# joshspeagle/brutus

Measured on AMD Instinct MI355X. Metric: stars/sec at 750k-model x 12-band grid; achieved HBM GB/s vs peak, higher is better.
Workload: dtype f64; 1 GPU; configs[1]: 750k-model x 12-band grid, Av-only solve (rvlim=(3.32,3.32)), no parallax; grid = synth.make_mist_like_grid (lattice-ordered like the MIST grid files); grid_generator=mist_like, nmodel=750000, nfilt=12, sub_batch=128, selected_models_last_sub_batch=44670752, streams_per_gpu=3, parallelism=stars sharded, 1 rank(s), no data-path collective

## Files before the change

brutus_amd/csrc/fit2_kernels.hpp:

```cpp
#pragma once

#include "fit_kernels.hpp"
#include "pre32_types.hpp"

namespace {

static_assert(PS_TILE == TILE && PS_NBMAX == NBMAX, "pre32_types.hpp and common.hpp disagree");

struct CallInit {
    int32_t *ids_all, *kfix, *k2, *counters;
    int ncounters;
};
__global__ void __launch_bounds__(64)
k_prep32(int nstar, const StarPrep *__restrict__ stars, float eps_scale, int dim_prior,
         Star32 *__restrict__ out, CallInit init) {
    static_assert(NBMAX <= 64, "one lane per band");
    __shared__ double s_a[NBMAX], s_b[NBMAX], s_c[NBMAX];
    __shared__ double s_gbar, s_D;
    __shared__ int s_bad;
    const int s = blockIdx.x, j = threadIdx.x;
    if (s >= nstar) return;
    if (init.ids_all && j == 0) {
        init.ids_all[s] = s;
        init.kfix[s] = 2;
// ... 316 lines not shown
            const float x = fmaxf(fmaxf(slot[0][threadIdx.x], slot[1][threadIdx.x]),
                                  fmaxf(slot[2][threadIdx.x], slot[3][threadIdx.x]));
            part[((int64_t)bx * nstar + s) * NV32 + v] = x;
        }
    }
}

__global__ void k_pre_decide(int nblkx, int nstar, const int32_t *__restrict__ star_ids,
                             const float *__restrict__ part, const Star32 *__restrict__ stars,
                             float ln_init, int rvf, int32_t *kfix,
                             int accept, float *__restrict__ st32, int32_t *__restrict__ k1,
                             int32_t *__restrict__ status, double *__restrict__ nomA,
                             int32_t *ctr, int32_t *__restrict__ probe_ids,
                             int32_t *__restrict__ redo_ids, const int32_t *nrun_dev) {
    __shared__ float sm[NV32][4];
    if (nrun_dev && (int)blockIdx.x >= *nrun_dev) return;
    const int s = star_ids[blockIdx.x];
    float v[NV32];
    for (int q = 0; q < NV32; ++q) v[q] = -INFINITY;
    for (int b = threadIdx.x; b < nblkx; b += blockDim.x) {
        const float *pp = part + ((int64_t)b * nstar + s) * NV32;
        for (int q = 0; q < NV32; ++q) v[q] = fmaxf(v[q], pp[q]);
    }
    for (int q = 0; q < NV32; ++q) {
        float x = v[q];
        for (int off = 32; off > 0; off >>= 1) x = fmaxf(x, __shfl_xor(x, off, 64));
        if ((threadIdx.x & 63) == 0) sm[q][threadIdx.x >> 6] = x;
    }
    __syncthreads();
    if (threadIdx.x != 0) return;
    for (int q = 0; q < NV32; ++q)
        v[q] = fmaxf(fmaxf(sm[q][0], sm[q][1]), fmaxf(sm[q][2], sm[q][3]));
    for (int q = 0; q < NV32; ++q) st32[(int64_t)s * NV32 + q] = v[q];
    const Star32 &sp = stars[s];
    const float ew = 2.f * sp.epsw;
    int st = 2, K1 = 0;
    const int K = kfix[s];
    if (sp.ok && !(v[8] > 0.f) && v[0] > -INFINITY) {
        const bool cont1 = v[1] > v[0] + ln_init + ew;
        const bool may1 = v[2] > v[0] + ln_init - ew;
        if (!may1) {
            K1 = 1;
            st = (rvf || K == 1) ? 0 : 1;
        } else if (cont1) {
            if (rvf) {
                K1 = 2;
                st = 0;
            } else if (K >= 2) {
                const bool cont2 = v[4] > v[3] + ln_init + ew;
                const bool may2 = v[5] > v[3] + ln_init - ew;
                if (!may2) {
                    K1 = 2;
                    st = (K == 2) ? 0 : 2;
                } else if (cont2) {
                    st = 2;
                }
            }
        }
    }
    if (!accept) {
        k1[s] = K1;
        status[s] = st;
        if (ctr) {
            if (st == 1) {
                kfix[s] = K1;
                redo_ids[atomicAdd(ctr + 1, 1)] = s;
            } else if (st == 2) {
                probe_ids[atomicAdd(ctr + 0, 1)] = s;
            }
        }
    }
    nomA[s] = (double)v[6] - 2. * (double)sp.eps;
}

template <int NB, bool RVF>
struct Tile64 {
    Coef<NB> c;
    double F0[NB];
    double R[RVF ? NB : 1];
};

template <int NB, bool RVF>
__device__ __forceinline__ void tile_load(const float *__restrict__ grid, int64_t nmodel_pad,
                                          int64_t i, double rv_mean, Tile64<NB, RVF> &t) {
    load_coef<NB>(grid, nmodel_pad, i, t.c);
    load_F0<NB>(grid, nmodel_pad, i, t.F0);
    if constexpr (RVF) coef_R<NB>(t.c, rv_mean, t.R);
}

template <int NB, bool RVF>
__device__ __forceinline__ void mag_phase(const Tile64<NB, RVF> &t, const StarPrep &sp,
                                          const DevParams &p, int K, double &av, double &rv) {
    av = p.av_mean;
    rv = p.rv_mean;
    if constexpr (RVF) {
        GramR Gm;
        gram_init_rf<NB>(t.c, t.R, sp, Gm);
        double a_, c_;
        if (K > 0) gram_sweep_rf(Gm, sp.S, p, av, a_, c_);
    } else {
        Gram Gm;
        gram_init<NB>(t.c, sp, Gm);
        for (int k = 0; k < K; ++k) {
            double a_, b_, c_;
            gram_sweep(Gm, sp.S, p, av, rv, a_, b_, c_);
        }
    }
}

template <int NB, bool RVF, bool FULL>
__device__ __forceinline__ void mle_at(const Tile64<NB, RVF> &t, const StarPrep &sp,
                                       const DevParams &p, double av, double rv,
                                       const double *__restrict__ tbl, Mle &m) {
    if constexpr (RVF) mle_fast_rf<NB, true, FULL ? 2 : 0>(t.c, t.R, t.F0, sp, p, av, tbl, m);
    else mle_fast<NB, true, FULL ? 2 : 0>(t.c, t.F0, sp, p, av, rv, tbl, m);
}

__device__ __forceinline__ void audit(float *__restrict__ aud, int s, float f32v, double f64v,
                                      double thr) {
    if (aud && f64v > thr - 12. && f32v == f32v) {
        const float d = fabsf((float)(f64v - (double)f32v));
        atomicMax(reinterpret_cast<int *>(aud + s), __float_as_int(d));
    }
}

__device__ __forceinline__ int64_t mword(int s, int ntile, int t, int w) {
    return (int64_t)s * (4 * ntile) + (int64_t)t * 4 + w;
}

__global__ void __launch_bounds__(256)
k_hot_list(int nblkx, int nstar, int mode, const float *__restrict__ part32,
           const double *__restrict__ nomA, const double *__restrict__ maxsurv,
           const Star32 *__restrict__ s32, double *__restrict__ nomB, double *__restrict__ part,
           int32_t *__restrict__ hot, int32_t *__restrict__ nhot) {
    const int s = blockIdx.x;
    double nm;
    if (mode == 0) {
        nm = nomA[s];
    } else {
        nm = maxsurv[s] - (double)s32[s].eps;
        if (threadIdx.x == 0) nomB[s] = nm;
    }
    for (int b = threadIdx.x; b < nblkx; b += blockDim.x) {
        const float *pp = part32 + ((int64_t)b * nstar + s) * NV32;
        const bool is_hot = !((double)pp[6 + mode] < nm) || pp[9] > 0.f;
        if (is_hot) hot[atomicAdd(nhot, 1)] = b * BRUTUS_MAX_BATCH + s;
        else part[(int64_t)b * nstar + s] = -INFINITY;
    }
}

template <int NB, bool RVF>
__global__ void __launch_bounds__(TILE, top_waves(NB))
k_top1(const float *__restrict__ grid, int64_t nmodel, int64_t nmodel_pad, int nstar,
       const StarPrep *__restrict__ stars, DevParams p, const int32_t *__restrict__ k1, int ntile,
       int mode, const float *__restrict__ plane32, const double *__restrict__ nom,
       const int32_t *__restrict__ hot, const int32_t *__restrict__ nhot,
       double *__restrict__ part, float *__restrict__ aud) {
    __shared__ double slot[4];
    __shared__ double s_tbl[64];
    const int n = *nhot;
    if ((int)blockIdx.x >= n) return;
    stage_exp_table(s_tbl);
    __syncthreads();
    const int lane = threadIdx.x & 63;
    for (int e = blockIdx.x; e < n; e += gridDim.x) {
        const int entry = hot[e];
        const int b = entry / BRUTUS_MAX_BATCH, s = entry - b * BRUTUS_MAX_BATCH;
        const int t0 = b * F2_T, t1 = min(ntile, t0 + F2_T);
        const StarPrep &sp = stars[s];
        const double nm_s = nom[s];
        const int K = k1[s];
        float v[F2_T];
#pragma unroll
        for (int u = 0; u < F2_T; ++u) {
            const int64_t i = (int64_t)(t0 + u) * TILE + threadIdx.x;
            v[u] = plane32[(int64_t)s * nmodel + (i < nmodel ? i : nmodel - 1)];
        }
        double mx = -INFINITY;
#pragma unroll
        for (int u = 0; u < F2_T; ++u) {
            const int64_t i = (int64_t)(t0 + u) * TILE + threadIdx.x;
            bool mine = t0 + u < t1 && i < nmodel && !((double)v[u] < nm_s);
            if (mode == 1 && mine) mine = !surv_is(v[u]);
            if (__ballot(mine) == 0ull) continue;
            Tile64<NB, RVF> tl;
            tile_load<NB, RVF>(grid, nmodel_pad, i, p.rv_mean, tl);
            double av, rv;
            mag_phase<NB, RVF>(tl, sp, p, K, av, rv);
            Mle m;
            mle_at<NB, RVF, false>(tl, sp, p, av, rv, s_tbl, m);
            double val;
            if (mode == 0) val = cull_stat(sp, m);
            else val = first_cut_lnprob(sp, final_lnl<false>(sp, p, m.chi2, false), m.scale, m.i00);
            if (mine) audit(aud, s, v[u], val, nm_s);
            if (mine && val == val) mx = val > mx ? val : mx;
        }
        block_max_store(mx, slot, part + (int64_t)b * nstar + s);
    }
}

__global__ void k_top_decide(int nblkx, int nstar, const int32_t *__restrict__ star_ids, int mode,
                             const double *__restrict__ part, const Star32 *__restrict__ s32,
                             double ln_thr, const double *__restrict__ maxsurv,
                             double *__restrict__ thr, double *__restrict__ cand) {
    __shared__ double sm[4];
    const int s = star_ids[blockIdx.x];
    double v = -INFINITY;
    for (int b = threadIdx.x; b < nblkx; b += blockDim.x) {
        const double x = part[(int64_t)b * nstar + s];
        v = x > v ? x : v;
    }
    v = wave_max(v);
    if ((threadIdx.x & 63) == 0) sm[threadIdx.x >> 6] = v;
    __syncthreads();
    if (threadIdx.x != 0) return;
    v = sm[0];
    for (int w = 1; w < 4; ++w) v = sm[w] > v ? sm[w] : v;
    if (mode == 0) {
        thr[s] = v + ln_thr;
        cand[s] = v + ln_thr - (double)s32[s].eps;
    } else {
        const double m = maxsurv[s] > v ? maxsurv[s] : v;
        thr[s] = m + ln_thr;
    }
}

__global__ void __launch_bounds__(TILE)
k_cmp_count32(int64_t nmodel, int ntile, const float *__restrict__ plane,
              const double *__restrict__ thr, int64_t *__restrict__ counts,
              unsigned long long *__restrict__ mask) {
    __shared__ int wsum[4];
    const int s = blockIdx.y, c = blockIdx.x;
    const int t0 = (int)((int64_t)ntile * c / NCHUNK), t1 = (int)((int64_t)ntile * (c + 1) / NCHUNK);
    const double th = thr[s];
    int n = 0;
#ifndef CNT_U
#define CNT_U 16
#endif
    constexpr int U = CNT_U;
    for (int tb = t0; tb < t1; tb += U) {
        float v[U];
#pragma unroll
        for (int u = 0; u < U; ++u) {
            const int64_t i = (int64_t)(tb + u) * TILE + threadIdx.x;
            const bool in = tb + u < t1 && i < nmodel;
            const float x = plane[(int64_t)s * nmodel + (in ? i : nmodel - 1)];
            v[u] = in ? x : -INFINITY;
        }
#pragma unroll
        for (int u = 0; u < U; ++u) {
            if (tb + u >= t1) break;
            const bool hit = !((double)v[u] < th);
            n += hit ? 1 : 0;
            const unsigned long long b = __ballot(hit);
            if ((threadIdx.x & 63) == 0)
                mask[(int64_t)s * (4 * ntile) + (int64_t)(tb + u) * 4 + (threadIdx.x >> 6)] = b;
        }
    }
#pragma unroll
    for (int off = 32; off > 0; off >>= 1) n += __shfl_xor(n, off, 64);
    if ((threadIdx.x & 63) == 0) wsum[threadIdx.x >> 6] = n;
    __syncthreads();
    if (threadIdx.x == 0) counts[(int64_t)s * NCHUNK + c] = wsum[0] + wsum[1] + wsum[2] + wsum[3];
}

__global__ void __launch_bounds__(TILE)
k_sel_classify(int64_t nmodel, int ntile, const Star32 *__restrict__ s32,
               const float *__restrict__ lnpr32,
               const double *__restrict__ lnprob_st, const int64_t *__restrict__ cand_off,
// ... 374 lines not shown
```

brutus_amd/csrc/fit_kernels.hpp:

```cpp
#pragma once

#include "common.hpp"
#include "fastmath.hpp"
#include "grid_kernels.hpp"

namespace {


struct Gram {
    double ua, ub, uy, aa, ab, bb, ay, by, yy;
};

template <int NB>
__device__ __forceinline__ void gram_init(const Coef<NB> &c, const StarPrep &sp, Gram &G) {
    double ua = 0., ub = 0., uy = 0., aa = 0., ab = 0., bb = 0., ay = 0., by = 0., yy = 0.;
#pragma unroll
    for (int j = 0; j < NB; ++j) {
        const double w = sp.iW[j];
        const double a = (double)c.r0[j], b = (double)c.dr[j];
        const double y = sp.g[j] - (double)c.m[j];
        const double aw = a * w, bw = b * w, yw = y * w;
        ua += aw;
        ub += bw;
        uy += yw;
// ... 260 lines not shown
    double s = s_num / s_den;
    if (s <= 1e-20) s = 1e-20;
    double SA = 0., SR = 0., AR = 0., AA = 0., RR = 0., AN = 0., RN = 0., chi2 = 0.;
    const double s2 = s + s;
    after = s;
#pragma unroll
    for (int j = 0; j < NB; ++j) {
        WIDE_ANCHOR(after, chi2);
        const double iv = sp.iV[j];
        const double f = Fc[j * TILE];
        const double D0 = wide_f64(c.dr[j], after);
        const double u = fma(rv, D0, wide_f64(c.r0[j], after)) * f;
        const double res = fma(-s, f, sp.d[j]);
        const double rw = res * iv, uw = u * iv;
        chi2 = fma(res, rw, chi2);
        AN = fma(u, rw, AN);
        AA = fma(u, uw, AA);
        if (LV >= 1) {
            const double v = D0 * f;
            const double vw = v * iv;
            RN = fma(v, rw, RN);
            RR = fma(v, vw, RR);
            if (LV >= 2) {
                const double t = fma(s2, f, -sp.d[j]);
                const double q = fma(-s, fast_exp10(-0.4 * wide_f64(c.m[j], after), tbl), t);
                SA = fma(uw, t, SA);
                SR = fma(vw, t, SR);
                AR = fma(vw, q, AR);
            }
        }
    }
    const double cs = fac * s, cs2 = cs * cs;
    double a_den = cs2 * AA, r_den = cs2 * RR;
    o.a_ss = a_den;
    o.r_ss = r_den;
    o.a_num = cs * AN;
    o.r_num = cs * RN;
    a_den += p.av_ivar;
    r_den += p.rv_ivar;
    a_den += p.a_reg;
    r_den += p.r_reg;
    o.scale = s;
    o.chi2 = chi2;
    o.i00 = s_den;
    o.i01 = fac * SA;
    o.i02 = fac * SR;
    o.i11 = a_den;
    o.i12 = cs * AR;
    o.i22 = r_den;
}

template <int NB>
__device__ __forceinline__ void gram_init_rf_wide(const Coef<NB> &c, double rv,
                                                  const StarPrep &sp, GramR &G) {
    double uR = 0., RR = 0., yR = 0., uy = 0., yy = 0.;
    double after = rv;
#pragma unroll
    for (int j = 0; j < NB; ++j) {
        WIDE_ANCHOR(after, yy);
        const double w = sp.iW[j];
        const double R = fma(rv, wide_f64(c.dr[j], after), wide_f64(c.r0[j], after));
        const double y = sp.g[j] - wide_f64(c.m[j], after);
        const double Rw = R * w, yw = y * w;
        uR += Rw;
        RR += R * Rw;
        yR += R * yw;
        uy += yw;
        yy += y * yw;
    }
    G.uR = uR; G.RR = RR; G.yR = yR; G.uy = uy; G.yy = yy;
}

template <int NB, bool RVF, bool FULL, int NR, int NF>
__device__ __forceinline__ void mle_list(const Coef<NB> &c, const double (&R)[NR],
                                         const double (&F0)[NF], LdsColumn Fc,
                                         const StarPrep &sp, const DevParams &p, double av,
                                         double rv, const double *__restrict__ tbl, Mle &o) {
    constexpr int LV = FULL ? 2 : RVF ? 0 : 1;
    if constexpr (wide_bands(NB)) mle_wide<NB, LV>(c, sp, p, av, rv, tbl, Fc, o);
    else if constexpr (RVF) mle_fast_rf<NB, true, LV>(c, R, F0, sp, p, av, tbl, o);
    else mle_fast<NB, true, LV>(c, F0, sp, p, av, rv, tbl, o);
}

template <int NB>
__device__ __forceinline__ void load_F0(const float *__restrict__ grid, int64_t nmodel_pad,
                                        int64_t i, double (&F0)[NB]) {
    const double *t = reinterpret_cast<const double *>(grid + (int64_t)6 * NB * nmodel_pad);
#pragma unroll
    for (int j = 0; j < NB; ++j) F0[j] = t[(int64_t)j * nmodel_pad + i];
}
template <int NB>
__device__ __forceinline__ void compute_F0_fast(const Coef<NB> &c, double (&F0)[NB]) {
#pragma unroll
    for (int j = 0; j < NB; ++j) F0[j] = poly_exp10(-0.4 * (double)c.m[j]);
}
template <int NB>
__device__ __forceinline__ void compute_F0_tbl(const Coef<NB> &c, const double *__restrict__ tbl,
                                               double (&F0)[NB]) {
#pragma unroll
    for (int j = 0; j < NB; ++j) F0[j] = fast_exp10(-0.4 * (double)c.m[j], tbl);
}

template <bool FASTLOG = false>
__device__ __forceinline__ double final_lnl(const StarPrep &sp, const DevParams &p, double chi2,
                                            bool survivor) {
    if (p.dim_prior)
        return chi2 > 0. ? sp.c0 + sp.c1 * (FASTLOG ? fast_log_r(chi2) : log(chi2)) - chi2 / 2.
                         : -INFINITY;
    return survivor ? -0.5 * chi2 + sp.lnl_const : -0.5 * chi2;
}
__device__ __forceinline__ double first_cut_lnprob(const StarPrep &sp, double lnl, double scale,
                                                   double i00) {
    double lnprob = lnl;
    if (sp.sp_on) {
        const double serr2 = 1. / fabs(i00);
        const double vt = sp.sp_var + serr2;
        const double ds = scale - sp.sp_mean;
        lnprob = lnl + -0.5 * (ds * ds / vt + log(2. * M_PI * vt));
    }
    if (!isfinite(lnprob)) lnprob = -BIG;
    return lnprob;
}

__device__ __forceinline__ double cull_stat(const StarPrep &sp, const Mle &m) {
    double lnlp = -0.5 * m.chi2;
    if (sp.has_par) {
        const double dp = sqrt(m.scale) - sp.par;
        lnlp -= 0.5 * (dp * dp * sp.par_ivar);
    }
    return lnlp;
}

template <int NB, int KS, bool RVF>
__global__ void __launch_bounds__(TILE)
k_k1probe(const float *__restrict__ grid, int64_t nmodel, int64_t nmodel_pad, int nstar, int nrun,
          const int32_t *__restrict__ star_ids, const StarPrep *__restrict__ stars, DevParams p,
          int tiles_per_block, int ntile, double *__restrict__ part,
          const int32_t *__restrict__ nrun_dev) {
    constexpr int NV = 2 * KS;
    __shared__ double slot[4];
    if (nrun_dev) nrun = *nrun_dev;
    for (int y = blockIdx.y; y < nrun; y += gridDim.y) {
    const int s = star_ids[y];
    const StarPrep &sp = stars[s];
    double mx[NV];
#pragma unroll
    for (int v = 0; v < NV; ++v) mx[v] = -INFINITY;
    const int t0 = blockIdx.x * tiles_per_block;
    const int t1 = min(ntile, t0 + tiles_per_block);
    for (int t = t0; t < t1; ++t) {
        const int64_t i = (int64_t)t * TILE + threadIdx.x;
        const bool live = i < nmodel;
        Coef<NB> c;
        load_coef<NB>(grid, nmodel_pad, i, c);
        double av = p.av_mean, rv = p.rv_mean;
        if constexpr (RVF) {
            double R[NB];
            coef_R<NB>(c, p.rv_mean, R);
            GramR G;
            gram_init_rf<NB>(c, R, sp, G);
            double dav, lw;
            gram_sweep_rf(G, sp.S, p, av, dav, lw);
            if (live && lw == lw) {
                mx[0] = lw > mx[0] ? lw : mx[0];
                if (fabs(dav) >= p.mtol) mx[1] = lw > mx[1] ? lw : mx[1];
#pragma unroll
                for (int k = 1; k < KS; ++k) mx[2 * k] = lw > mx[2 * k] ? lw : mx[2 * k];
            }
        } else {
            Gram G;
            gram_init<NB>(c, sp, G);
#pragma unroll
            for (int k = 0; k < KS; ++k) {
// ... 237 lines not shown
        if (item >= end) {
            c += 8;
            seek();
        }
    }
};

constexpr int CONT_P = 16;
struct SegWalk {
    int item, end;
    __device__ __forceinline__ void init(const int32_t *wbase, int nstar, const int32_t *act, int nact,
                                         int unit) {
        const int c = unit % NCHUNK, a = (unit / NCHUNK) % nact;
        const int piece = unit / (NCHUNK * nact);
        const int e = c * nstar + act[a];
        end = wbase[e + 1];
        item = wbase[e] + piece;
        if (item >= end) item = -1;
    }
    __device__ __forceinline__ bool done() const { return item < 0; }
    __device__ __forceinline__ void next() {
        item += CONT_P;
        if (item >= end) item = -1;
    }
};

template <int NB>
__device__ __forceinline__ void gather_coef(const float *__restrict__ grid, int64_t nmodel_pad,
                                            int64_t i, Coef<NB> &c) {
    const float4 *row =
        reinterpret_cast<const float4 *>(grid + (int64_t)3 * NB * nmodel_pad + i * (3 * NB));
    float t[3 * NB];
#pragma unroll
    for (int q = 0; q < 3 * NB / 4; ++q) {
        const float4 v = row[q];
        t[4 * q] = v.x;
        t[4 * q + 1] = v.y;
        t[4 * q + 2] = v.z;
        t[4 * q + 3] = v.w;
    }
#pragma unroll
    for (int j = 0; j < NB; ++j) {
        c.m[j] = t[3 * j];
        c.r0[j] = t[3 * j + 1];
        c.dr[j] = t[3 * j + 2];
    }
}

typedef float f32x4 __attribute__((ext_vector_type(4)));
template <int NB>
struct RowRegs {
    f32x4 q[3 * NB / 4];
};
template <int NB>
__device__ __forceinline__ void gather_row(const float *__restrict__ grid, int64_t nmodel_pad,
                                           int64_t i, RowRegs<NB> &r) {
    const f32x4 *row =
        reinterpret_cast<const f32x4 *>(grid + (int64_t)3 * NB * nmodel_pad + i * (3 * NB));
#pragma unroll
    for (int q = 0; q < 3 * NB / 4; ++q) r.q[q] = row[q];
}
template <int NB>
__device__ __forceinline__ void row_to_coef(const RowRegs<NB> &r, Coef<NB> &c) {
    float t[3 * NB];
#pragma unroll
    for (int q = 0; q < 3 * NB / 4; ++q) {
        t[4 * q] = r.q[q].x;
        t[4 * q + 1] = r.q[q].y;
        t[4 * q + 2] = r.q[q].z;
        t[4 * q + 3] = r.q[q].w;
    }
#pragma unroll
    for (int j = 0; j < NB; ++j) {
        c.m[j] = t[3 * j];
        c.r0[j] = t[3 * j + 1];
        c.dr[j] = t[3 * j + 2];
    }
}
template <int NB>
__device__ __forceinline__ void landed(RowRegs<NB> &r) {
#pragma unroll
    for (int q = 0; q < 3 * NB / 4; ++q) {
        f32x4 t = r.q[q];
        asm volatile("" : "+v"(t) : : "memory");
        r.q[q] = t;
    }
}
__device__ __forceinline__ void landed(int32_t &x) {
    int32_t t = x;
    asm volatile("" : "+v"(t) : : "memory");
    x = t;
}

struct RecPlanes {
    double *vals;
    int64_t cap;
    __device__ __forceinline__ double *plane(int v) const { return vals + (int64_t)v * cap; }
};

template <int NB, bool RVF, bool FIRST>
__global__ void __launch_bounds__(TILE, fflux_waves(NB, FIRST))
k_fflux(const float *__restrict__ grid, int64_t nmodel, int64_t nmodel_pad, int nstar,
        const StarPrep *__restrict__ stars, DevParams p, const int32_t *__restrict__ k1,
        const int32_t *__restrict__ k2state, const int32_t *__restrict__ cand_idx,
        const int64_t *__restrict__ cand_off, const int32_t *__restrict__ wbase,
        const ItemGeom *__restrict__ items, RecPlanes rec, double *__restrict__ step_st,
        double *__restrict__ lnprob_st, double *__restrict__ part, float *__restrict__ surv32,
        const double *__restrict__ thr_cull, const int32_t *__restrict__ act, int nact,
        const int32_t *__restrict__ nact_dev, int run) {
    if (!FIRST && nact_dev) nact = *nact_dev;
    if (!FIRST && nact <= 0) return;
    __shared__ double s_tbl[64];
    stage_exp_table(s_tbl);
    __syncthreads();
    constexpr bool WIDE = wide_bands(NB);
    __shared__ double s_F[WIDE ? NB * TILE : 1];
    const LdsColumn Fc = (LdsColumn)s_F + (WIDE ? threadIdx.x : 0);
    constexpr int niter = FIRST ? 2 : 1;
    int s_nxt = 0;
    auto lane_model = [&](int item) -> int32_t {
        const ItemGeom ig = items[item < 0 ? 0 : item];
        s_nxt = ig.s;
        const int64_t q = ig.q0 + threadIdx.x;
        const int64_t last = ig.q0 + ig.n - 1;
        return cand_idx[q < last ? q : last];
    };
    double *__restrict__ r_lnl = rec.plane(0), *__restrict__ r_chi2 = rec.plane(1),
                        *__restrict__ r_scale = rec.plane(2), *__restrict__ r_av = rec.plane(3),
                        *__restrict__ r_rv = rec.plane(4);
    auto walk = [&](auto &wk) {
    int32_t i_nxt = lane_model(wk.item);
    constexpr bool PER_STAR = FIRST && NB <= 12;
    double aL = -INFINITY, aT = -INFINITY, aM = -INFINITY;
    while (!wk.done()) {
        const int item = wk.item;
        wk.next();
        const ItemGeom ig = items[item];
        const int s = ig.s;
        const int32_t i_me = i_nxt;
        i_nxt = lane_model(wk.item);
        if (k2state[s] < 0) {
            landed(i_nxt);
            continue;
        }
        const StarPrep &sp = stars[s];
        const int64_t q = ig.q0 + threadIdx.x;
        const bool live = (int)threadIdx.x < ig.n && q < rec.cap;
        double L = -INFINITY, T = -INFINITY, M = -INFINITY;
        bool go = live;
        const int64_t i = i_me;
        const int64_t o = (int64_t)s * nmodel + i;
        if (!FIRST && live) go = surv_is(surv32[o]);
        Mle m;
        double o_lnl = 0., o_lnprob = 0., o_av = 0., o_rv = 0., o_step = 0.;
        bool store = false;
        if (go) {
            Coef<NB> c;
            gather_coef<NB>(grid, nmodel_pad, i, c);
            double F0[WIDE ? 1 : NB];
#ifdef BRUTUS_F0_FROM_TABLE
            if constexpr (!WIDE) load_F0<NB>(grid, nmodel_pad, i, F0);
#else
            if constexpr (!WIDE) compute_F0_tbl<NB>(c, s_tbl, F0);
#endif
            double av, rv, step, lnl_old;
            double R[RVF && !WIDE ? NB : 1];
            if constexpr (RVF && !WIDE) coef_R<NB>(c, p.rv_mean, R);
            if constexpr (FIRST) {
                av = p.av_mean;
                rv = p.rv_mean;
                const int K = k1[s];
                if constexpr (RVF) {
                    GramR G;
                    if constexpr (WIDE) gram_init_rf_wide<NB>(c, p.rv_mean, sp, G);
                    else gram_init_rf<NB>(c, R, sp, G);
                    for (int k = 0; k < K; ++k) {
                        double a_, c_;
                        gram_sweep_rf(G, sp.S, p, av, a_, c_);
                    }
                } else {
                    Gram G;
                    gram_init<NB>(c, sp, G);
                    for (int k = 0; k < K; ++k) {
                        double a_, b_, c_;
                        gram_sweep(G, sp.S, p, av, rv, a_, b_, c_);
                    }
                }
                step = 1.0;
                lnl_old = -BIG;
            } else {
                av = r_av[q];
                rv = RVF ? p.rv_mean : r_rv[q];
                step = step_st[q];
                lnl_old = -0.5 * r_chi2[q];
            }
            mle_list<NB, RVF, false>(c, R, F0, Fc, sp, p, av, rv, s_tbl, m);
            if constexpr (FIRST) {
                go = cull_stat(sp, m) > thr_cull[s];
                if (go) surv32[o] = surv_tag(q - cand_off[s]);
            }
            double lnl_new = lnl_old, dl = 0.;
            for (int it = 0; go && it < niter; ++it) {
                double dav = (m.a_num + (p.av_mean - av) * p.av_ivar) / (m.a_ss + p.av_ivar) * step;
                if (dav < p.avmin - av) dav = p.avmin - av;
                if (dav > p.avmax - av) dav = p.avmax - av;
                av += dav;
                if constexpr (RVF) {
                    if (it + 1 < niter) mle_list<NB, RVF, false>(c, R, F0, Fc, sp, p, av, rv, s_tbl, m);
                    else mle_list<NB, RVF, true>(c, R, F0, Fc, sp, p, av, rv, s_tbl, m);
                } else {
                    double drv = (m.r_num + (p.rv_mean - rv) * p.rv_ivar) / (m.r_ss + p.rv_ivar) * step;
                    if (drv < p.rvmin - rv) drv = p.rvmin - rv;
                    if (drv > p.rvmax - rv) drv = p.rvmax - rv;
                    rv += drv;
                    constexpr bool SHORT_FIRST = NB != 16;
                    if (SHORT_FIRST && it + 1 < niter) mle_list<NB, RVF, false>(c, R, F0, Fc, sp, p, av, rv, s_tbl, m);
                    else mle_list<NB, RVF, true>(c, R, F0, Fc, sp, p, av, rv, s_tbl, m);
                }
                lnl_new = -0.5 * m.chi2;
                dl = fabs(lnl_new - lnl_old);
                if (lnl_new < lnl_old) step /= 1.2;
                lnl_old = lnl_new;
            }
            if (go) {
                o_lnl = final_lnl<RVF>(sp, p, m.chi2, true);
                o_lnprob = first_cut_lnprob(sp, o_lnl, m.scale, m.i00);
                o_av = av;
                o_rv = rv;
                o_step = step;
                M = o_lnprob;
                if (lnl_new == lnl_new) {
                    L = lnl_new;
                    if (dl > p.ltol) T = lnl_new;
                }
            }
            store = go;
        }
        landed(i_nxt);
        if (store) {
#define FF_ST(p, x) __builtin_nontemporal_store((x), (p) + q)
            FF_ST(r_lnl, o_lnl);
            FF_ST(r_chi2, m.chi2);
            FF_ST(r_scale, m.scale);
            FF_ST(r_av, o_av);
            if constexpr (!RVF) FF_ST(r_rv, o_rv);
            FF_ST(rec.plane(5), m.i00);
            FF_ST(rec.plane(6), m.i01);
// ... 107 lines not shown
    __shared__ unsigned long long s_word[3][TILE];
    __shared__ unsigned long long s_pre[TILE];
    const int s = blockIdx.y, c = blockIdx.x;
    const int t0 = (int)((int64_t)ntile * c / NCHUNK), t1 = (int)((int64_t)ntile * (c + 1) / NCHUNK);
    int64_t base = offsets[(int64_t)s * NCHUNK + c];
    int64_t dbase = doffsets[(int64_t)s * NCHUNK + c] + cand_off[nstar];
    int64_t cbase = coffsets[(int64_t)s * NCHUNK + c];
    const int lane = threadIdx.x & 63, w = threadIdx.x >> 6;
    const unsigned long long below = (1ull << lane) - 1ull;
    const int64_t row = (int64_t)s * (4 * ntile);
    constexpr unsigned long long F20 = (1ull << 20) - 1ull;
    for (int tb = t0; tb < t1; tb += TILE / 4) {
        const int nt = min(TILE / 4, t1 - tb);
        const bool in = (int)threadIdx.x < 4 * nt;
        const int64_t a = row + (int64_t)tb * 4 + (in ? threadIdx.x : 0);
        unsigned long long wm = mask[a], wd = dmask[a], wc = cmask[a];
        if (!in) wm = wd = wc = 0ull;
        unsigned long long tot;
        const unsigned long long pre = block_exclusive_sum<unsigned long long, TILE>(
            (unsigned long long)__popcll(wm) | ((unsigned long long)__popcll(wd) << 20) |
                ((unsigned long long)__popcll(wc) << 40),
            s_slot, tot);
        s_word[0][threadIdx.x] = wm;
        s_word[1][threadIdx.x] = wd;
        s_word[2][threadIdx.x] = wc;
        s_pre[threadIdx.x] = pre;
        __syncthreads();
#pragma unroll 4
        for (int k = 0; k < nt; ++k) {
            const unsigned long long b = s_word[0][4 * k + w];
            if ((b >> lane) & 1ull) {
                const unsigned long long bd = s_word[1][4 * k + w], bc = s_word[2][4 * k + w];
                const unsigned long long pk = s_pre[4 * k + w];
                const int32_t i = (int32_t)((int64_t)(tb + k) * TILE + threadIdx.x);
                const int64_t r = base + (int64_t)(pk & F20) + __popcll(b & below);
                int64_t slot;
                if ((bd >> lane) & 1ull) {
                    slot = dbase + (int64_t)((pk >> 20) & F20) + __popcll(bd & below);
                    der_idx[slot - cand_off[nstar]] = i;
                } else {
                    slot = cbase + (int64_t)(pk >> 40) + __popcll(bc & below);
                }
                if (r < capacity) {
                    rec_idx[r] = i;
                    rec_slot[r] = (int32_t)slot;
                }
            }
        }
        base += (int64_t)(tot & F20);
        dbase += (int64_t)((tot >> 20) & F20);
        cbase += (int64_t)(tot >> 40);
        __syncthreads();
    }
}

template <int NB, bool RVF>
__global__ void __launch_bounds__(TILE, list_waves(NB))
k_derive(const float *__restrict__ grid, int64_t nmodel_pad, int nstar,
         const StarPrep *__restrict__ stars, DevParams p, const int32_t *__restrict__ k1,
         const int32_t *__restrict__ der_idx, const int32_t *__restrict__ wbase,
         const ItemGeom *__restrict__ items, const int64_t *__restrict__ cand_off,
         RecPlanes rec, int run) {
    __shared__ double s_tbl[64];
    stage_exp_table(s_tbl);
    __syncthreads();
    constexpr bool WIDE = wide_bands(NB);
    __shared__ double s_F[WIDE ? NB * TILE : 1];
    const LdsColumn Fc = (LdsColumn)s_F + (WIDE ? threadIdx.x : 0);
    auto lane_model = [&](int item) -> int32_t {
        if (item < 0) return 0;
        const ItemGeom ig = items[item];
        const int64_t q = ig.q0 + threadIdx.x;
        const int64_t last = ig.q0 + ig.n - 1;
        return der_idx[q < last ? q : last];
    };
    const int64_t slot0 = cand_off[nstar];
    ItemWalk wk;
    wk.init(wbase, nstar, blockIdx.x & 7, blockIdx.x >> 3, (gridDim.x + 7 - (blockIdx.x & 7)) >> 3, run);
    if (wk.done()) return;
    int item = wk.item;
    wk.next();
    int item1 = wk.item;
    constexpr bool PIPE = NB <= 12;
    int32_t i0 = lane_model(item), i1 = lane_model(item1);
    RowRegs<NB> nx;
    if (PIPE) gather_row<NB>(grid, nmodel_pad, i0, nx);
    landed(i1);
    if (PIPE) landed<NB>(nx);
    while (item >= 0) {
        Coef<NB> c;
        if (PIPE) {
            row_to_coef<NB>(nx, c);
            gather_row<NB>(grid, nmodel_pad, i1, nx);
        } else {
            gather_row<NB>(grid, nmodel_pad, i0, nx);
            row_to_coef<NB>(nx, c);
        }
        if (item1 >= 0) wk.next();
        const int item2 = item1 >= 0 ? wk.item : -1;
        int32_t i2 = lane_model(item2);
        const ItemGeom ig = items[item];
        const int s = ig.s;
        const int64_t slot = slot0 + ig.q0 + threadIdx.x;
        const bool live = (int)threadIdx.x < ig.n && slot < rec.cap;
        const bool wave_live = (int)(threadIdx.x & ~63u) < ig.n;
        double o_lnl = 0., o_av = 0., o_rv = 0.;
        Mle m;
        if (wave_live) {
            const StarPrep &sp = stars[s];
            double F0[WIDE ? 1 : NB];
#ifdef BRUTUS_F0_FROM_TABLE
            if constexpr (!WIDE) load_F0<NB>(grid, nmodel_pad, i0, F0);
#else
            if constexpr (!WIDE) compute_F0_tbl<NB>(c, s_tbl, F0);
#endif
            double av = p.av_mean, rv = p.rv_mean;
            const int K = k1[s];
            if constexpr (RVF) {
                double R[WIDE ? 1 : NB];
                GramR G;
                if constexpr (WIDE) {
                    gram_init_rf_wide<NB>(c, rv, sp, G);
                } else {
                    coef_R<NB>(c, rv, R);
                    gram_init_rf<NB>(c, R, sp, G);
                }
                double a_, c_;
                if (K > 0) gram_sweep_rf(G, sp.S, p, av, a_, c_);
                mle_list<NB, true, true>(c, R, F0, Fc, sp, p, av, rv, s_tbl, m);
            } else {
                Gram G;
                gram_init<NB>(c, sp, G);
                for (int kk = 0; kk < K; ++kk) {
                    double a_, b_, c_;
                    gram_sweep(G, sp.S, p, av, rv, a_, b_, c_);
                }
                const double R1[1] = {0.};
                mle_list<NB, false, true>(c, R1, F0, Fc, sp, p, av, rv, s_tbl, m);
            }
            o_lnl = final_lnl<RVF>(sp, p, m.chi2, false);
            o_av = av;
            o_rv = rv;
        }
        if (PIPE) landed<NB>(nx);
        landed(i2);
        if (wave_live && live) {
            double *out = rec.vals + slot;
#define REC_ST(k, x) __builtin_nontemporal_store((x), out + (int64_t)(k) * rec.cap)
            REC_ST(0, o_lnl);
            REC_ST(1, m.chi2);
            REC_ST(2, m.scale);
            REC_ST(3, o_av);
            if constexpr (!RVF) REC_ST(4, o_rv);
            REC_ST(5, m.i00);
            REC_ST(6, m.i01);
            REC_ST(7, m.i02);
            REC_ST(8, m.i11);
            REC_ST(9, m.i12);
            REC_ST(10, m.i22);
#undef REC_ST
        }
        item = item1;
        item1 = item2;
        i0 = i1;
        i1 = i2;
    }
}

}
```

brutus_amd/csrc/grid_kernels.hpp:

```cpp
#pragma once

#include "common.hpp"
#include "fastmath.hpp"

namespace {

template <int NB>
struct MagState {
    double res[NB], R[NB];
    double av, rv, P, Q;
    double dav, drv, logwt;
};

template <int NB>
__device__ __forceinline__ void mag_init(const Coef<NB> &c, const StarPrep &sp,
                                         const DevParams &p, double av0, double rv0,
                                         MagState<NB> &st) {
    st.av = av0;
    st.rv = rv0;
    double P = 0., Q = 0.;
#pragma unroll
    for (int j = 0; j < NB; ++j) {
        const double D = (double)c.dr[j];
        const double R = (double)c.r0[j] + st.rv * D;
// ... 159 lines not shown
        pe = perr[s];
    }
    const bool fin = isfinite(p) && isfinite(pe);
    sp.has_par = fin ? 1 : 0;
    sp.par = fin ? p : 0.;
    sp.par_ivar = fin ? 1. / (pe * pe) : 0.;
    sp.sp_on = (fin && p / pe > 4.) ? 1 : 0;
    const double pm = p > 0. ? p : 0.;
    sp.sp_mean = sp.sp_on ? pm * pm + pe * pe : 0.;
    sp.sp_var = sp.sp_on ? 2. * pe * pe * pe * pe + 4. * pm * pm * pe * pe : 0.;
}

__global__ void __launch_bounds__(64)
k_prep(int nstar, int nfilt, const double *__restrict__ flux,
       const double *__restrict__ err, const uint8_t *__restrict__ mask,
       const double *__restrict__ par, const double *__restrict__ perr,
       int has_parallax, StarPrep *__restrict__ out, int32_t *__restrict__ ndim_out) {
    static_assert(NBMAX <= 64, "one lane per band");
    __shared__ double s_w[NBMAX], s_lnv[NBMAX], s_d2[NBMAX];
    __shared__ int s_ok[NBMAX];
    const int s = blockIdx.x, j = threadIdx.x;
    if (s >= nstar) return;
    StarPrep &sp = out[s];
    const double kmag = 2.5 / log(10.);
    if (j < NBMAX) {
        double d = 0., iv = 0., g = 0., iw = 0., lnv = 0., d2 = 0.;
        bool ok = false;
        if (j < nfilt) {
            const double f = flux[(int64_t)s * nfilt + j];
            const double e = err[(int64_t)s * nfilt + j];
            ok = mask[(int64_t)s * nfilt + j] && isfinite(f) && isfinite(e) && e > 0.;
            if (ok) {
                const double v = e * e;
                d = f;
                iv = 1. / v;
                lnv = log(v);
                g = -2.5 * log10(f);
                double W = kmag * kmag * v / (f * f);
                if (!isfinite(g)) {
                    g = 0.;
                    W = 1e50;
                }
                iw = 1. / W;
                d2 = f * f * iv;
            }
        }
        sp.d[j] = d;
        sp.iV[j] = iv;
        sp.g[j] = g;
        sp.iW[j] = iw;
        s_w[j] = iw;
        s_lnv[j] = lnv;
        s_d2[j] = d2;
        s_ok[j] = ok ? 1 : 0;
    }
    __syncthreads();
    if (j != 0) return;
    int ndim = 0;
    double S = 0., sumlnv = 0., D2 = 0.;
    for (int k = 0; k < NBMAX; ++k) {
        if (!s_ok[k]) continue;
        ++ndim;
        sumlnv += s_lnv[k];
        S += s_w[k];
        D2 += s_d2[k];
    }
    sp.S = S;
    sp.D2 = D2;
    sp.ndim = ndim;
    sp.lnl_const = -0.5 * (ndim * log(2. * M_PI) + sumlnv);
    const double df = (double)(ndim - 3);
    sp.c0 = -log(exp2(df / 2.) * tgamma(df / 2.));
    sp.c1 = df / 2. - 1.;
    prep_parallax(sp, has_parallax, par, perr, s);
    sp.pad_ = 0;
    ndim_out[s] = ndim;
}

__global__ void k_relayout(const float *__restrict__ aos, int64_t nmodel, int nfilt, int nb,
                           int64_t nmodel_pad, float *__restrict__ blob) {
    const int64_t i = (int64_t)blockIdx.x * blockDim.x + threadIdx.x;
    if (i >= nmodel_pad) return;
    float *rows = blob + (int64_t)3 * nb * nmodel_pad;
    double *f0_soa = reinterpret_cast<double *>(blob + (int64_t)6 * nb * nmodel_pad);
    for (int j = 0; j < nb; ++j) {
        float m = 0.f;
        for (int k = 0; k < 3; ++k) {
            float v = 0.f;
            if (i < nmodel && j < nfilt) v = aos[(i * nfilt + j) * 3 + k];
            if (k == 0) m = v;
            blob[(int64_t)(3 * j + k) * nmodel_pad + i] = v;
            rows[(i * nb + j) * 3 + k] = v;
        }
        const double f0 = fast_exp10(-0.4 * (double)m);
        f0_soa[(int64_t)j * nmodel_pad + i] = f0;
    }
}

template <int NB>
__global__ void __launch_bounds__(TILE)
k_mag_stats(const float *__restrict__ grid, int64_t nmodel, int64_t nmodel_pad, int nstar,
            const StarPrep *__restrict__ stars, DevParams p, int kmax,
            double *__restrict__ part, const double *__restrict__ av_init,
            const double *__restrict__ rv_init) {
    __shared__ double slot[4];
    const int64_t i = (int64_t)blockIdx.x * TILE + threadIdx.x;
    const bool live = i < nmodel;
    Coef<NB> c;
    load_coef<NB>(grid, nmodel_pad, i, c);
    const double av0 = av_init ? av_init[live ? i : nmodel - 1] : p.av_mean;
    const double rv0 = rv_init ? rv_init[live ? i : nmodel - 1] : p.rv_mean;
    const int s0 = blockIdx.y * STAR_GROUP;
    const int s1 = min(nstar, s0 + STAR_GROUP);
    const double ninf = -INFINITY;
    for (int s = s0; s < s1; ++s) {
        const StarPrep &sp = stars[s];
        MagState<NB> st;
        mag_init<NB>(c, sp, p, av0, rv0, st);
        double *out = part + ((int64_t)blockIdx.x * nstar + s) * (2 * kmax);
        for (int k = 0; k < kmax; ++k) {
            mag_sweep<NB>(c, sp, p, st);
            const double lw = (live && st.logwt == st.logwt) ? st.logwt : ninf;
            const bool big = (fabs(st.dav) >= p.mtol) || (fabs(st.drv) >= p.mtol);
            block_max_store(lw, slot, out + 2 * k);
            block_max_store(big ? lw : ninf, slot, out + 2 * k + 1);
        }
    }
}

__global__ void k_reduce_decide(int mode, int ntile, int nstar, int nval,
                                const double *__restrict__ part, double thresh,
                                double *__restrict__ vmax, int32_t *__restrict__ iters,
                                int32_t *__restrict__ n_unconv) {
    __shared__ double sm[KCAP * 2][4];
    const int s = blockIdx.x;
    double v[KCAP * 2];
    for (int q = 0; q < nval; ++q) v[q] = -INFINITY;
    for (int t = threadIdx.x; t < ntile; t += blockDim.x) {
        const double *pp = part + ((int64_t)t * nstar + s) * nval;
        for (int q = 0; q < nval; ++q) v[q] = pp[q] > v[q] ? pp[q] : v[q];
    }
    for (int q = 0; q < nval; ++q) {
        const double m = wave_max(v[q]);
        if ((threadIdx.x & 63) == 0) sm[q][threadIdx.x >> 6] = m;
    }
    __syncthreads();
    if (threadIdx.x != 0) return;
    for (int q = 0; q < nval; ++q) {
        double m = sm[q][0];
        for (int w = 1; w < 4; ++w) m = sm[q][w] > m ? sm[q][w] : m;
        v[q] = m;
    }
    if (mode == 0) {
        int K1 = 0;
        for (int k = 0; k < nval / 2; ++k) {
            const double L = v[2 * k] > -BIG ? v[2 * k] : -BIG;
            const double T = v[2 * k + 1];
            const bool unconv = T > L + thresh;
            if (!unconv) {
                K1 = k + 1;
                break;
            }
        }
        iters[s] = K1;
        if (K1 == 0) atomicAdd(n_unconv, 1);
    } else if (mode == 1) {
        vmax[s] = v[0];
    } else {
        const bool unconv = v[1] > v[0] + thresh;
        if (iters[s] >= 0) {
            if (unconv) {
                iters[s] += 1;
                atomicAdd(n_unconv, 1);
            } else {
                iters[s] = -iters[s] - 1;
            }
        }
    }
// ... 135 lines not shown
```

Before: 39900 stars/s.

## Store precomputed F0 row-major and gather it per model with 16-byte loads

Switches the precomputed F0 table from structure-of-arrays to one row per model, so a single model's fluxes can be read as 16-byte vector loads. It adds a pipelined F0 gather next to the coefficient-row prefetch in the record kernel, and routes the tile kernel to compute F0 from the LDS exp table for NB<=12 instead of loading it. Several of the new paths are behind a macro level whose default is 0, so the default build mostly just changes the layout and the tile-kernel F0 source. The cost traded is extra HBM traffic against extra exp arithmetic.

```diff
diff --git a/brutus_amd/csrc/fit2_kernels.hpp b/brutus_amd/csrc/fit2_kernels.hpp
--- a/brutus_amd/csrc/fit2_kernels.hpp
+++ b/brutus_amd/csrc/fit2_kernels.hpp
@@ -422,9 +422,16 @@
 
 template <int NB, bool RVF>
 __device__ __forceinline__ void tile_load(const float *__restrict__ grid, int64_t nmodel_pad,
-                                          int64_t i, double rv_mean, Tile64<NB, RVF> &t) {
+                                          int64_t i, double rv_mean,
+                                          const double *__restrict__ tbl, Tile64<NB, RVF> &t) {
     load_coef<NB>(grid, nmodel_pad, i, t.c);
-    load_F0<NB>(grid, nmodel_pad, i, t.F0);
+#ifdef BRUTUS_F0_TILE_TABLE
+    constexpr bool ROWS = true;
+#else
+    constexpr bool ROWS = NB > 12;
+#endif
+    if constexpr (ROWS) load_F0<NB>(grid, nmodel_pad, i, t.F0);
+    else compute_F0_tbl<NB>(t.c, tbl, t.F0);
     if constexpr (RVF) coef_R<NB>(t.c, rv_mean, t.R);
 }
 
@@ -524,7 +531,7 @@
             if (mode == 1 && mine) mine = !surv_is(v[u]);
             if (__ballot(mine) == 0ull) continue;
             Tile64<NB, RVF> tl;
-            tile_load<NB, RVF>(grid, nmodel_pad, i, p.rv_mean, tl);
+            tile_load<NB, RVF>(grid, nmodel_pad, i, p.rv_mean, s_tbl, tl);
             double av, rv;
             mag_phase<NB, RVF>(tl, sp, p, K, av, rv);
             Mle m;
diff --git a/brutus_amd/csrc/fit_kernels.hpp b/brutus_amd/csrc/fit_kernels.hpp
--- a/brutus_amd/csrc/fit_kernels.hpp
+++ b/brutus_amd/csrc/fit_kernels.hpp
@@ -366,13 +366,42 @@
     else mle_fast<NB, true, LV>(c, F0, sp, p, av, rv, tbl, o);
 }
 
+typedef double f64x2 __attribute__((ext_vector_type(2)));
+template <int NB>
+struct F0Regs {
+    f64x2 q[NB / 2];
+};
+template <int NB>
+__device__ __forceinline__ void gather_F0(const float *__restrict__ grid, int64_t nmodel_pad,
+                                          int64_t i, F0Regs<NB> &r) {
+    static_assert(NB % 2 == 0, "a row of F0 is read in 16-byte pieces");
+    const f64x2 *row = reinterpret_cast<const f64x2 *>(
+        reinterpret_cast<const double *>(grid + (int64_t)6 * NB * nmodel_pad) + i * NB);
+#pragma unroll
+    for (int q = 0; q < NB / 2; ++q) r.q[q] = row[q];
+}
+template <int NB>
+__device__ __forceinline__ void F0_from_regs(const F0Regs<NB> &r, double (&F0)[NB]) {
+#pragma unroll
+    for (int q = 0; q < NB / 2; ++q) {
+        F0[2 * q] = r.q[q].x;
+        F0[2 * q + 1] = r.q[q].y;
+    }
+}
 template <int NB>
 __device__ __forceinline__ void load_F0(const float *__restrict__ grid, int64_t nmodel_pad,
                                         int64_t i, double (&F0)[NB]) {
-    const double *t = reinterpret_cast<const double *>(grid + (int64_t)6 * NB * nmodel_pad);
-#pragma unroll
-    for (int j = 0; j < NB; ++j) F0[j] = t[(int64_t)j * nmodel_pad + i];
-}
+    F0Regs<NB> r;
+    gather_F0<NB>(grid, nmodel_pad, i, r);
+    F0_from_regs<NB>(r, F0);
+}
+#ifndef BRUTUS_F0_FROM_TABLE
+#define BRUTUS_F0_FROM_TABLE 0
+#endif
+constexpr bool fflux_f0_from_table(int nb, bool first) {
+    return BRUTUS_F0_FROM_TABLE >= (first ? 1 : 2) && !wide_bands(nb) && !(nb == 16 && first);
+}
+constexpr bool derive_f0_from_table(int nb) { return BRUTUS_F0_FROM_TABLE >= 3 && !wide_bands(nb); }
 template <int NB>
 __device__ __forceinline__ void compute_F0_fast(const Coef<NB> &c, double (&F0)[NB]) {
 #pragma unroll
@@ -776,6 +805,15 @@
 #pragma unroll
     for (int q = 0; q < 3 * NB / 4; ++q) {
         f32x4 t = r.q[q];
+        asm volatile("" : "+v"(t) : : "memory");
+        r.q[q] = t;
+    }
+}
+template <int NB>
+__device__ __forceinline__ void landed(F0Regs<NB> &r) {
+#pragma unroll
+    for (int q = 0; q < NB / 2; ++q) {
+        f64x2 t = r.q[q];
         asm volatile("" : "+v"(t) : : "memory");
         r.q[q] = t;
     }
@@ -852,11 +890,8 @@
             Coef<NB> c;
             gather_coef<NB>(grid, nmodel_pad, i, c);
             double F0[WIDE ? 1 : NB];
-#ifdef BRUTUS_F0_FROM_TABLE
-            if constexpr (!WIDE) load_F0<NB>(grid, nmodel_pad, i, F0);
-#else
-            if constexpr (!WIDE) compute_F0_tbl<NB>(c, s_tbl, F0);
-#endif
+            if constexpr (!WIDE && fflux_f0_from_table(NB, FIRST)) load_F0<NB>(grid, nmodel_pad, i, F0);
+            else if constexpr (!WIDE) compute_F0_tbl<NB>(c, s_tbl, F0);
             double av, rv, step, lnl_old;
             double R[RVF && !WIDE ? NB : 1];
             if constexpr (RVF && !WIDE) coef_R<NB>(c, p.rv_mean, R);
@@ -1130,19 +1165,35 @@
     wk.next();
     int item1 = wk.item;
     constexpr bool PIPE = NB <= 12;
+    constexpr bool F0TBL = !WIDE && derive_f0_from_table(NB);
+#ifdef BRUTUS_F0_AT_ITEM
+    constexpr bool F0PIPE = false;
+#else
+    constexpr bool F0PIPE = PIPE && F0TBL;
+#endif
     int32_t i0 = lane_model(item), i1 = lane_model(item1);
     RowRegs<NB> nx;
+    F0Regs<F0TBL ? NB : 2> fx;
     if (PIPE) gather_row<NB>(grid, nmodel_pad, i0, nx);
+    if constexpr (F0PIPE) gather_F0<NB>(grid, nmodel_pad, i0, fx);
     landed(i1);
     if (PIPE) landed<NB>(nx);
+    if constexpr (F0PIPE) landed(fx);
     while (item >= 0) {
         Coef<NB> c;
+        double F0[WIDE ? 1 : NB];
         if (PIPE) {
             row_to_coef<NB>(nx, c);
+            if constexpr (F0PIPE) F0_from_regs<NB>(fx, F0);
             gather_row<NB>(grid, nmodel_pad, i1, nx);
+            if constexpr (F0PIPE) gather_F0<NB>(grid, nmodel_pad, i1, fx);
         } else {
             gather_row<NB>(grid, nmodel_pad, i0, nx);
             row_to_coef<NB>(nx, c);
+        }
+        if constexpr (F0TBL && !F0PIPE) {
+            gather_F0<NB>(grid, nmodel_pad, i0, fx);
+            F0_from_regs<NB>(fx, F0);
         }
         if (item1 >= 0) wk.next();
         const int item2 = item1 >= 0 ? wk.item : -1;
@@ -1156,12 +1207,7 @@
         Mle m;
         if (wave_live) {
             const StarPrep &sp = stars[s];
-            double F0[WIDE ? 1 : NB];
-#ifdef BRUTUS_F0_FROM_TABLE
-            if constexpr (!WIDE) load_F0<NB>(grid, nmodel_pad, i0, F0);
-#else
-            if constexpr (!WIDE) compute_F0_tbl<NB>(c, s_tbl, F0);
-#endif
+            if constexpr (!WIDE && !F0TBL) compute_F0_tbl<NB>(c, s_tbl, F0);
             double av = p.av_mean, rv = p.rv_mean;
             const int K = k1[s];
             if constexpr (RVF) {
@@ -1191,6 +1237,7 @@
             o_rv = rv;
         }
         if (PIPE) landed<NB>(nx);
+        if constexpr (F0PIPE) landed(fx);
         landed(i2);
         if (wave_live && live) {
             double *out = rec.vals + slot;
diff --git a/brutus_amd/csrc/grid_kernels.hpp b/brutus_amd/csrc/grid_kernels.hpp
--- a/brutus_amd/csrc/grid_kernels.hpp
+++ b/brutus_amd/csrc/grid_kernels.hpp
@@ -265,7 +265,7 @@
     const int64_t i = (int64_t)blockIdx.x * blockDim.x + threadIdx.x;
     if (i >= nmodel_pad) return;
     float *rows = blob + (int64_t)3 * nb * nmodel_pad;
-    double *f0_soa = reinterpret_cast<double *>(blob + (int64_t)6 * nb * nmodel_pad);
+    double *f0_rows = reinterpret_cast<double *>(blob + (int64_t)6 * nb * nmodel_pad);
     for (int j = 0; j < nb; ++j) {
         float m = 0.f;
         for (int k = 0; k < 3; ++k) {
@@ -276,7 +276,7 @@
             rows[(i * nb + j) * 3 + k] = v;
         }
         const double f0 = fast_exp10(-0.4 * (double)m);
-        f0_soa[(int64_t)j * nmodel_pad + i] = f0;
+        f0_rows[i * nb + j] = f0;
     }
 }
 
```

After: 39890 stars/s, median of 2. No clear change (-0.0%).
